# tsy935/eeg-gnn-ssl

Measured on AMD Instinct MI355X. Metric: EEG clips/sec (60s, 19ch, K=2, 2-layer x64) fwd+bwd, higher is better.
Workload: dtype f32

## Files before the change

### eeg_gnn_ssl_amd/csrc/api.cpp

```cpp
#include <algorithm>
#include <atomic>
#include <cmath>
#include <cstdarg>
#include <cstdio>
#include <cstring>

#include <string>
#include <vector>

#include "../../include/eeg_dcrnn.h"
#include "../../include/eeg_dcrnn_dev.h"
#include "../../include/eeg_dcrnn_prof.h"
#include "kernels_decoder.h"
#include "diffuse_launch.h"
#include "kernels_diffuse.h"
#include "kernels_eval.h"
#include "kernels_moments.h"
#include "kernels_scan.h"
#include "kernels_resample.h"
#include "kernels_edf.h"
#include "kernels_occlude.h"
#include "kernels_data.h"
#include "kernels_records.h"
#include "kernels_feat.h"
// ... 674 lines not shown
                                 void* stream) {
    if (eeg_dcrnn_spectral_pack_floats(Fin, H, M, N) == 0)
        return fail("pack_cell_spectral: input_dim=%d rnn_units=%d hop matrices=%d nodes=%d: the spectral form exists for 64 units", Fin, H, M, N);
    if (Wg == nullptr || Wc == nullptr || basis == nullptr || spack == nullptr) return fail("pack_cell_spectral: null pointer");
    if (launch_spec_pack(Wg, Wc, basis, Fin, H, M, N, spack, S_(stream))) return fail("pack_cell_spectral: launch failed");
    return check_launch("pack_cell_spectral");
}
int eeg_dcrnn_pack_cells(int n_cells, const float* const* Wg, const float* const* bg, const float* const* Wc, const float* const* bc,
                         const int32_t* Fin, int H, int M, float* const* packs, const float* basis, int N, float* const* spacks,
                         void* stream) {
    if (n_cells < 1 || n_cells > 4) return fail("pack_cells: %d cells (1..4 per launch)", n_cells);
    if (Wg == nullptr || bg == nullptr || Wc == nullptr || bc == nullptr || Fin == nullptr || packs == nullptr) return fail("pack_cells: null pointer table");
    if (!seq_h_supported(H)) return fail("pack_cells: rnn_units=%d unsupported", H);
    if (!seq_m_supported(M)) return fail("pack_cells: num hop matrices M=%d unsupported (1,2,3,4,5,7)", M);
    if ((basis == nullptr) != (spacks == nullptr)) return fail("pack_cells: the per-frequency packs need the basis block and their output table");
    int fin[4];
    for (int c = 0; c < n_cells; ++c) {
        fin[c] = Fin[c];
        if (fin[c] < 4 || fin[c] % 4 != 0) return fail("pack_cells: input dim %d of cell %d must be a positive multiple of 4", fin[c], c);
        if (Wg[c] == nullptr || bg[c] == nullptr || Wc[c] == nullptr || bc[c] == nullptr || packs[c] == nullptr || (spacks != nullptr && spacks[c] == nullptr))
            return fail("pack_cells: null pointer in the tables of cell %d", c);
        if (spacks != nullptr && eeg_dcrnn_spectral_pack_floats(fin[c], H, M, N) == 0)
            return fail("pack_cells: input_dim=%d rnn_units=%d hop matrices=%d nodes=%d: the spectral form exists for 64 units", fin[c], H, M, N);
    }
    if (launch_pack_cells(n_cells, Wg, bg, Wc, bc, fin, H, M, packs, basis, N, spacks, S_(stream))) return fail("pack_cells: launch failed");
    return check_launch("pack_cells");
}
int eeg_dcrnn_spectral_ok(const eeg_layer_dims* d, int need_dx) {
    if (!layer_dims_positive(d) || d->p_batched) return 0;
    if (d->x_planes_ready && d->Fin != d->H) return 0;
    if (check_dims(d->N, d->H, d->Fin, d->M)) return 0;
    return spec_supported(d->T, d->B, d->N, d->H, d->Fin, d->M, need_dx) ? 1 : 0;
}

int eeg_dcrnn_batch_major_ok(const eeg_layer_dims* d) {
    if (!diffuse_streams(diffuse_call(false, d->p_batched, d->T * d->B, d->B, d->N, d->Fin, d->M))) return 0;
    const int R = d->T * d->B * d->N;
    const GemmKnobs k = gemm_knobs();
    return (nn_dma_applies(d->Fin, R, 3 * d->H, k) && tn_dma_applies(d->Fin, 3 * d->H, k)) ? 2 : 1;
}

int eeg_dcrnn_layer_fwd(const eeg_layer_dims* d, const float* X, float* Xtm, const float* h0, const float* P,
                        const float* pack, float* planes, float* Hext, float* Rs, float* Us, float* Cs, float* RHs,
                        float* Hplanes, float* RHplanes, float* ws, void* stream) {
    if (check_dims(d->N, d->H, d->Fin, d->M)) return 1;
    if (d->T < 1 || d->B < 1) return fail("layer_fwd: empty sequence/batch (T=%d, B=%d)", d->T, d->B);
    const bool save = Rs != nullptr;
    if (save != (Us != nullptr) || save != (Cs != nullptr) || save != (RHs != nullptr))
        return fail("layer_fwd: Rs/Us/Cs/RHs must be all NULL or all non-NULL");
    hipStream_t st = S_(stream);
    const int S = d->T * d->B, R = S * d->N, H = d->H, M = d->M, Fin = d->Fin;
    const size_t state = (size_t)d->B * d->N * H;
    CellPack p = make_cell_pack(Fin, H, M);
    if (h0 != nullptr && h0 != Hext && copy_floats(Hext, h0, state, st)) return 1;
    const size_t xs = d->x_plane_stride > 0 ? (size_t)d->x_plane_stride : (size_t)R * Fin;
    BtMap bt;
    if (d->x_batch_major) {
        if (Xtm != nullptr || d->x_planes_ready) return fail("layer_fwd: x_batch_major excludes Xtm and x_planes_ready");
        if (d->spectral == nullptr && eeg_dcrnn_batch_major_ok(d) != 2) return fail("layer_fwd: x_batch_major is not available for this shape (eeg_dcrnn_batch_major_ok)");
        bt.T = d->T; bt.B = d->B; bt.N = d->N;
    }
    float* XW = ws;
    if (d->spectral != nullptr) {
        if (!eeg_dcrnn_spectral_ok(d, 0)) return fail("layer_fwd: the spectral form does not cover this shape (eeg_dcrnn_spectral_ok)");
        if (Xtm != nullptr || d->spack == nullptr) return fail("layer_fwd: spectral excludes Xtm and needs spack");
        if ((Hplanes != nullptr) != (RHplanes != nullptr)) return fail("layer_fwd: Hplanes/RHplanes must be both NULL or both non-NULL");
        const SpecPack sp = make_spec_pack(Fin, H, M, d->N);
        const int N = d->N, Sp = spec_rows(S), SpE = d->B + Sp;
        const size_t xgs = d->x_plane_stride > 0 ? (size_t)d->x_plane_stride : (size_t)Sp * Fin;
        float* Yh = ws + (size_t)R * 3 * H;
        if (!d->x_planes_ready && spec_mix(1, X, d->spectral, N, d->T, d->B, Fin, d->x_batch_major ? 1 : 0, planes, st, "spec_mix_x")) return 1;
        const SpecNnPlan nn = spec_nn_plan(Fin, Sp, N, sp.nct_x, num_cus(), spec_knobs());
        if (spec_plan_error("layer_fwd (spectral x-part)", nn.error)) return 1;
        const bool regs = nn.kind == SpecNnKind::Regs;
        if (launch_spec_nn(nn, planes, xgs, Fin, Sp, N, d->spack + (regs ? sp.sxr : sp.sxq), regs ? sp.sxr_stride : sp.sxq_stride, Yh, st, "gemm_nn_xw",
                           pack + p.bias, d->spectral + spec_csum_offset(N))) return fail("gemm_nn (spectral): launch failed");
        SeqFwdArgs a{XW, h0 != nullptr ? Hext : nullptr, P, d->p_batched, pack + p.bhg, pack + p.bhc, Hext + state, Rs, Us, Cs, RHs, nullptr, nullptr,
                     (size_t)0, d->T, d->B, N, d->act, seq_probe_arg(st)};
        SeqCall call = seq_fwd_call(H, M, N, d->T, d->B, 0, a.probe);
        call.spectral = true; call.Sp = Sp; call.SpE = SpE;
        const SeqPlan plan = seq_fwd_plan(call);
        if (plan.kind == SeqKind::TwoWaveSpec) {
            a.XW = Yh; a.Hpl = Hplanes; a.RHpl = RHplanes; a.spec_U = d->spectral; a.spec_Sp = Sp; a.spec_SpE = SpE;
            if (seq_fwd(H, M, plan, a, st)) return 1;
            if (Hplanes != nullptr) {
                if (launch_spec_zero_rows(Hplanes, N, (d->T + 1) * d->B, SpE, H, st)) return fail("spec_zero_rows: launch failed");
                if (launch_spec_zero_pad(RHplanes, N, S, H, st)) return fail("spec_zero_pad: launch failed");
            }
        } else {
            if (spec_mix(0, Yh, d->spectral, N, d->T, d->B, 3 * H, 0, XW, st, "spec_mix_y")) return 1;
            if (seq_fwd(H, M, plan, a, st)) return 1;
            if (Hplanes != nullptr) {
                if (spec_mix(1, Hext, d->spectral, N, d->T + 1, d->B, H, 0, Hplanes, st, "spec_mix_h", SpE)) return 1;
                if (spec_mix(1, RHs, d->spectral, N, d->T, d->B, H, 0, RHplanes, st, "spec_mix_h")) return 1;
            }
        }
        return check_launch("layer_fwd (spectral)");
    } else if (d->x_planes_ready) {
        if (Xtm != nullptr) return fail("layer_fwd: x_planes_ready excludes a batch-major input");
    } else {
        if (diffuse_fwd(X, P, d->p_batched, S, d->B, d->N, Fin, M, planes, st, xs, d->x_batch_major ? 2 : (Xtm != nullptr ? 1 : 0), Xtm)) return 1;
        if (Xtm != nullptr) X = Xtm;
    }
    SegPtrs segs;
    for (int m = 0; m < kMaxM; ++m) segs.p[m] = m == 0 ? X : (m < M ? planes + (size_t)(m - 1) * xs : nullptr);
    const bool bf3 = d->pack3 != nullptr && pack3_supported(Fin, H, M);
    const Pack3 q = make_pack3(Fin, H, M);
    const NnCall cxw = nn_call(M, Fin, R, 3 * H / 16, 3 * H, 3 * H, bt, p.has_bxq, bf3 ? q.xw_nct : 0);
    if (gemm_nn(gemm_nn_plan(cxw), cxw, segs, NnRhs{pack + p.bx, pack + p.bxq, bf3 ? d->pack3 + q.xw : nullptr}, pack + p.bias, XW, st, "gemm_nn_xw", bt)) return 1;
    if ((Hplanes != nullptr) != (RHplanes != nullptr)) return fail("layer_fwd: Hplanes/RHplanes must be both NULL or both non-NULL");
    SeqFwdArgs a{XW, h0 != nullptr ? Hext : nullptr, P, d->p_batched, pack + p.bhg, pack + p.bhc, Hext + state, Rs, Us, Cs, RHs, Hplanes, RHplanes,
                 (size_t)(d->T + 1) * state, d->T, d->B, d->N, d->act, seq_probe_arg(st)};
    return seq_fwd(H, M, seq_fwd_plan(seq_fwd_call(H, M, d->N, d->T, d->B, a.plane_stride, a.probe)), a, st);
}

size_t eeg_dcrnn_layer_bwd_ws_floats(const eeg_layer_dims* d, int need_dx) { return layer_dims_positive(d) ? bwd_ws(d, need_dx).total : 0; }

int eeg_dcrnn_layer_bwd(const eeg_layer_dims* d, const float* X, const float* P, const float* pack,
                        const float* planes, const float* Hext, const float* Rs, const float* Us, const float* Cs,
                        const float* RHs, const float* Hplanes, const float* RHplanes, const float* dHseq,
                        const float* d_at_end, const float* d_at_len,
                        const int64_t* lengths, float* dX, float* dh0, float* dWg, float* dbg, float* dWc,
                        float* dbc, float* ws, void* stream) {
    if (check_dims(d->N, d->H, d->Fin, d->M)) return 1;
    if (d->T < 1 || d->B < 1) return fail("layer_bwd: empty sequence/batch (T=%d, B=%d)", d->T, d->B);
    hipStream_t st = S_(stream);
    const int S = d->T * d->B, R = S * d->N, H = d->H, M = d->M, Fin = d->Fin, N = d->N;
    const size_t state = (size_t)d->B * N * H;
    CellPack p = make_cell_pack(Fin, H, M);
    BwdWs w = bwd_ws(d, dX != nullptr);
    float* dXW = ws + w.dxw;
    float* dbias = ws + w.dbias;
    SeqBwdArgs a{Hext + state, Hext, Rs, Us, Cs, dHseq, d_at_end, d_at_len,
                 reinterpret_cast<const long long*>(lengths), P, d->p_batched, pack + p.b1, pack + p.b2,
                 dXW, dh0, dbias, d->T, d->B, N, d->act, seq_probe_arg(st)};
    SeqCall call = seq_bwd_call(H, M, N, d->T, d->B, a.probe);
    call.spectral = d->spectral != nullptr; call.Sp = spec_rows(S); call.SpE = d->B + spec_rows(S);
    const SeqPlan plan = seq_bwd_plan(call);
    const bool dyh_done = plan.kind == SeqKind::TwoWaveSpec;
    if (dyh_done) { a.spec_U = d->spectral; a.dYh = ws + w.dyh; a.spec_Sp = call.Sp; }
    if (seq_bwd(H, M, plan, a, st)) return 1;
    const size_t xs = d->x_plane_stride > 0 ? (size_t)d->x_plane_stride : (size_t)R * Fin;
    BtMap bt;
    if (d->x_batch_major) {
        if (d->spectral == nullptr && eeg_dcrnn_batch_major_ok(d) != 2) return fail("layer_bwd: x_batch_major is not available for this shape");
        bt.T = d->T; bt.B = d->B; bt.N = N;
    }
    if (d->spectral != nullptr) {
        if (!eeg_dcrnn_spectral_ok(d, dX != nullptr)) return fail("layer_bwd: the spectral form does not cover this shape (eeg_dcrnn_spectral_ok)");
        if (d->spack == nullptr) return fail("layer_bwd: spectral needs spack");
        if ((Hplanes != nullptr) != (RHplanes != nullptr)) return fail("layer_bwd: Hplanes/RHplanes must be both NULL or both non-NULL");
        const SpecPack sp = make_spec_pack(Fin, H, M, N);
        const int Sp = spec_rows(S), SpE = d->B + Sp;
        float* dYh = ws + w.dyh;
        if (dyh_done) {
            if (launch_spec_zero_pad(dYh, N, S, 3 * H, st)) return fail("spec_zero_pad: launch failed");
        } else if (spec_mix(1, dXW, d->spectral, N, d->T, d->B, 3 * H, 0, dYh, st, "spec_mix_dy")) return 1;
        const float *hh = Hplanes, *rhh = RHplanes;
        size_t hh_gs = (size_t)SpE * H;
        if (hh == nullptr) {
            if (spec_mix(1, Hext, d->spectral, N, d->T, d->B, H, 0, ws + w.hplanes, st, "spec_mix_h")) return 1;
            if (spec_mix(1, RHs, d->spectral, N, d->T, d->B, H, 0, ws + w.rhplanes, st, "spec_mix_h")) return 1;
            hh = ws + w.hplanes; rhh = ws + w.rhplanes; hh_gs = 0;
        }
        if (cell_weight_grads_spectral(d, planes, xs_spec(d), hh, hh_gs, rhh, dYh, ws + w.partial, w, dWg, dWc, st, dbias, dbg, dbc)) return 1;
        if (dX != nullptr) {
// ... 1304 lines not shown
```

### eeg_gnn_ssl_amd/csrc/kernels_seq.h

```cpp
#pragma once
#include "common.h"
#include "lds_diffuse.h"

namespace eeg {

constexpr int seq_nks(int N) { return N <= 20 ? 5 : 8; }
constexpr bool seq_has_two_wave(int H, int M, int nks) { return H == 64 && nks == 5 && M <= 3; }
constexpr bool seq_has_spec(int H, int M, int nks) { return seq_has_two_wave(H, M, nks) && M >= 2; }
constexpr bool seq_has_probe(int H, int M, int nks) { return kDevBuild && H == 64 && M == 3 && nks == 5; }
constexpr bool seq_has_stream(int H, int M) { return H == 64 && M <= 5; }

template <int H, int M>
struct SeqGeom {
    static constexpr int KA = M * H, KAP = lds_stride_x(KA), KS = KA / 4;
    static constexpr int KG = M * 2 * H, KGP = lds_stride_x(KG), KSG = KG / 4;
    static constexpr int NGT = 2 * H / 16, NCT = H / 16;
    static constexpr int GT = ceil_div(NGT, 4), CT = ceil_div(NCT, 4);
};
constexpr size_t seq_fwd_lds_floats(int H, int M) { return (size_t)(M - 1) * kPFloats + 2 * 32 * lds_stride_x(M * H); }
constexpr size_t seq_fwd2_lds_floats(int H, int M, bool spec) {
    return seq_fwd_lds_floats(H, M) + 16 * 64 + (spec ? 3 * 16 * 64 + 4 * 64 + 4 * (M * H / 4 / 4) * 256 : 0);
}
constexpr size_t seq_bwd_lds_floats(int H, int M, int rows) {
    return (size_t)(M - 1) * kPFloats + (size_t)rows * (lds_stride_x(M * H) + lds_stride_x(M * 2 * H));
// ... 428 lines not shown
                    f32x4 rh = rg * ld4(A + lds_sw(node[nt], col, KAP));
                    rh = valid[nt] ? rh : zero4;
                    st4(A2 + lds_sw(node[nt], col, KAP), rh);
                    if (save && valid[nt]) {
                        wbuf_st4(bR, oh[i][nt], 0u, rg);
                        wbuf_st4(bRH, oh[i][nt], 0u, rh);
                        wbuf_st4(bU, oh[i][nt], 0u, u);
                    }
                }
            }
        }
        pp.mark(2);
        diffuse_own(A2, RHpl, t);
        pp.mark(7);
        EEG_LDS_BARRIER();
        pp.mark(3);
        if (t + 1 < T) fetch_xw(t + 1);

        mfma_nodes32<CT, KS, REM4, 0, 0, false, false, REM4>(A2, KAP, lane, lr, lg, wc, ac);
        pp.mark(4);
        const wbuf_t bH = make_wbuf(Hseq + s * N * H), bC = make_wbuf((save ? Cs : Hseq) + s * N * H);
#pragma unroll
        for (int i = 0; i < CT; ++i) {
            const int ct = wave + 4 * i;
            if (ct < NCT) {
                const int col = ct * 16 + 4 * lg;
#pragma unroll
                for (int nt = 0; nt < 2; ++nt) {
                    if (REM4 && nt == 1) {
                        const float u1 = ug[i][1][0], h1 = A[l1[i]];
                        const float c1 = act == 0 ? tanhf_(ac[i][1][0]) : fmaxf(ac[i][1][0], 0.f);
                        const float hn1 = valid1 ? u1 * h1 + (1.f - u1) * c1 : 0.f;
                        A[l1[i]] = hn1;
                        if (valid1) {
                            wbuf_st1(bH, oh[i][1], 0u, hn1);
                            if (save) wbuf_st1(bC, oh[i][1], 0u, c1);
                        }
                        continue;
                    }
                    const f32x4 u = ug[i][nt], h = ld4(A + lds_sw(node[nt], col, KAP));
                    const f32x4 c = act == 0 ? tanh4_(ac[i][nt]) : relu4_(ac[i][nt]);
                    f32x4 hn = u * h + (1.f - u) * c;
                    hn = valid[nt] ? hn : zero4;
                    st4(A + lds_sw(node[nt], col, KAP), hn);
                    if (valid[nt]) {
                        wbuf_st4(bH, oh[i][nt], 0u, hn);
                        if (save) wbuf_st4(bC, oh[i][nt], 0u, c);
                    }
                }
            }
        }
        pp.mark(5);
        if (t + 1 < T || Hpl != nullptr) diffuse_own(A, Hpl, t + 1);
        pp.mark(6);
    }
    }
    pp.dump(probe, 0);
}

template <int H, int M, int NKS, bool PROBE = false, bool SPEC = false>
__global__ __launch_bounds__(512, 1) void seq_fwd2_kernel(
    const float* __restrict__ XW, const float* __restrict__ h0, const float* __restrict__ P, int p_batched,
    const float* __restrict__ bhg, const float* __restrict__ bhc,
    float* __restrict__ Hseq, float* __restrict__ Rs, float* __restrict__ Us, float* __restrict__ Cs,
    float* __restrict__ RHs, float* __restrict__ Hpl, float* __restrict__ RHpl, size_t plane_stride,
    int T, int B, int N, int act, long long* probe, const float* __restrict__ spec_U = nullptr, int spec_Sp = 0, int spec_SpE = 0) {
    using G = SeqGeom<H, M>;
    PhaseProbe<PROBE> pp;
    pp.start();
    static_assert(G::CT == 1 && NKS == 5, "one column tile per wave, second node tile on the 4x4x1 MFMA");
    constexpr int KAP = G::KAP, KS = G::KS, NGT = G::NGT, NCT = G::NCT, UST = 64;
    EEG_DYN_SMEM(sm);
    float* Pl = sm;
    float* A = Pl + (M - 1) * kPFloats;
    float* A2 = A + 32 * KAP;
    const int tid = threadIdx.x, lane = tid & 63, wave8 = SPEC ? wave_uniform(tid >> 6) : (tid >> 6), role = wave8 >> 2, wave = wave8 & 3;
    const int lr = lane & 15, lg = lane >> 4;
    float* U = A2 + 32 * KAP;
    float* XR = U + 16 * UST;
    float* XC = XR + 16 * UST;
    float* XRr = XC + 2 * 16 * UST;
    float* W1L = XRr + 4 * 64;
    const bool save = Rs != nullptr;
    const int ct = wave;
    const wbuf_t bH = make_wbuf(Hseq), bR = make_wbuf(save ? Rs : Hseq), bU = make_wbuf(save ? Us : Hseq),
                 bC = make_wbuf(save ? Cs : Hseq), bRH = make_wbuf(save ? RHs : Hseq);

    float w0[1][KS], w1[1][KS];
#pragma unroll
    for (int ks = 0; ks < KS; ++ks) w0[0][ks] = bhg[((size_t)ks * NGT + (role == 0 ? ct : NCT + ct)) * 64 + lane];
    if (!SPEC || role == 0) {
#pragma unroll
        for (int ks = 0; ks < KS; ++ks) w1[0][ks] = bhc[((size_t)ks * NCT + ct) * 64 + lane];
    } else {
#pragma unroll
        for (int q = 0; q < KS / 4; ++q) {
            f32x4 v;
#pragma unroll
            for (int j = 0; j < 4; ++j) v[j] = bhc[((size_t)(4 * q + j) * NCT + ct) * 64 + lane];
            st4(W1L + (ct * (KS / 4) + q) * 256 + 4 * lane, v);
        }
    }
    auto clip = [&](const int b, auto ROLE_T) __attribute__((always_inline)) {
    constexpr int ROLE_C = decltype(ROLE_T)::value;
    __syncthreads();
    for (int e = tid; e < 2 * 32 * KAP; e += 512) A[e] = 0.f;
    lds_load_polys(Pl, P, p_batched ? b : 0, M, N);
    __syncthreads();
    if (h0 != nullptr) {
        for (int e = tid; e < N * H; e += 512) A[lds_sw(e / H, e % H, KAP)] = h0[(size_t)b * N * H + e];
    } else {
        for (int e = tid; e < N * H; e += 512) (Hseq - (size_t)B * N * H)[(size_t)b * N * H + e] = 0.f;
    }
    __syncthreads();

    const bool valid[2] = {lr < N, 16 + lr < N};
    const int nodec[2] = {valid[0] ? lr : N - 1, valid[1] ? 16 + lr : N - 1};
    const f32x4 zero4 = {0.f, 0.f, 0.f, 0.f};
    const int col = ct * 16 + 4 * lg;
    const int oxw0 = nodec[0] * (3 * H) + col, oh0 = nodec[0] * H + col;
    const int node1 = 16 + lg, col1 = ct * 16 + lr;
    const bool valid1 = node1 < N;
    const int oxw1 = (valid1 ? node1 : N - 1) * (3 * H) + col1, oh1 = (valid1 ? node1 : N - 1) * H + col1;
    const int l1 = lds_sw(node1, col1, KAP);
    if (ROLE_C < 0 ? role == 0 : ROLE_C == 0) {
        EEG_SETPRIO(3);
        float pf[poly_slots<M, NKS>()][NKS];
        load_poly_frags<M, NKS, false>(Pl, pf, lr, lg);
        auto diffuse_own = [&](float* buf, float* planes, int t) {
            EEG_WAVE_SYNC();
            float* g = (!SPEC && planes != nullptr) ? planes + ((size_t)t * B + b) * N * H : nullptr;
            lds_diffuse_tile<M, NKS>(buf, KAP, ct * 16, H, pf, lr, lg, g, plane_stride, N, true);
        };
        diffuse_own(A, Hpl, 0);
        f32x4 nxr0 = zero4, nxc = zero4;
        float nxr1 = 0.f;
        auto fetch_xw = [&](int t) {
            if constexpr (SPEC) return;
            const wbuf_t bx = make_wbuf(XW + ((size_t)t * B + b) * N * (3 * H));
            nxr0 = wbuf_ld4(bx, oxw0, 0u);
            nxr1 = wbuf_ld(bx, oxw1, 0u);
            nxc = wbuf_ld4(bx, oxw0 + 2 * H, 0u);
        };
        fetch_xw(0);
        pp.stamp(1);
        pp.last = PROBE ? cycle_now() : 0;
        ClockSample cs;
        const bool cs_me = !PROBE && b == 0 && tid == 0;
        cs.begin(probe, cs_me);
        constexpr int QSA = KS / 4 / M;
        f32x4 rc[5] = {zero4, zero4, zero4, zero4, zero4};
        f32x4 ra = zero4;
        bool pre_r = false;
        for (int t = 0; t < T; ++t) {
            const size_t s = (size_t)t * B + b;
            f32x4 ar[1][2] = {{nxr0, (f32x4){nxr1, 0.f, 0.f, 0.f}}}, ac[1][2] = {{nxc, zero4}};
            const unsigned so = (unsigned)(s * N * H);
            EEG_LDS_BARRIER();
            pp.mark(0);
            if constexpr (SPEC) {
                ar[0][0] = ld4(XR + lds_sw(lr, col, UST));
                ar[0][1][0] = XRr[ct * 64 + lane];
                if (M > 1 && pre_r) ra += ar[0][0];
            }

            if (M > 1 && pre_r) {
                ar[0][0] = ra;
                mfma_nodes32<1, KS, true, 0, 0, false, true, true, (M > 1 ? QSA : 0)>(A, KAP, lane, lr, lg, w0, ar, rc);
            } else
                mfma_nodes32<1, KS, true, 0, 0, false, true, true>(A, KAP, lane, lr, lg, w0, ar);
            pp.mark(1);
            {
                const f32x4 rg = sigmoid4_(ar[0][0]);
                f32x4 rh = rg * ld4(A + lds_sw(lr, col, KAP));
                rh = valid[0] ? rh : zero4;
                st4(A2 + lds_sw(lr, col, KAP), rh);
                const float rg1 = sigmoidf_(ar[0][1][0]);
                const float rh1 = valid1 ? rg1 * A[l1] : 0.f;
                A2[l1] = rh1;
                if (save && valid[0]) {
                    wbuf_st4(bR, oh0, so, rg);
                    wbuf_st4(bRH, oh0, so, rh);
                }
                if (save && valid1) {
                    wbuf_st1(bR, oh1, so, rg1);
                    wbuf_st1(bRH, oh1, so, rh1);
                }
            }
            pp.mark(2);
            diffuse_own(A2, RHpl, t);
            pp.mark(7);
            EEG_LDS_BARRIER();
            pp.mark(3);
            if (t + 1 < T) fetch_xw(t + 1);
            if constexpr (SPEC) ac[0][0] = ld4(XC + (t & 1) * (16 * UST) + lds_sw(lr, col, UST));
            mfma_nodes32<1, KS, true, 1>(A2, KAP, lane, lr, lg, w1, ac);
            pp.mark(4);
            {
                const f32x4 u = ld4(U + lds_sw(lr, col, UST)), h = ld4(A + lds_sw(lr, col, KAP));
                const f32x4 c = act == 0 ? tanh4_(ac[0][0]) : relu4_(ac[0][0]);
                f32x4 hn = u * h + (1.f - u) * c;
                hn = valid[0] ? hn : zero4;
                st4(A + lds_sw(lr, col, KAP), hn);
                if (valid[0]) {
                    wbuf_st4(bH, oh0, so, hn);
                    if (save) wbuf_st4(bC, oh0, so, c);
                }
            }
            pp.mark(5);
            EEG_LDS_BARRIER();
            if (t + 1 < T || (!SPEC && Hpl != nullptr)) diffuse_own(A, Hpl, t + 1);
            pre_r = M > 1 && t + 1 < T;
            if (pre_r) {
                ra = SPEC ? zero4 : nxr0;
                rc[0] = rc[1] = rc[2] = rc[3] = rc[4] = zero4;
                f32x4 rr4[4] = {zero4, zero4, zero4, zero4};
                mfma_tile_quads<KS, 0, QSA>(A, KAP, lane, lr, lg, w0[0], ra, rc[4], rr4);
                rc[0] = rr4[0]; rc[1] = rr4[1]; rc[2] = rr4[2]; rc[3] = rr4[3];
            }
            pp.mark(6);
        }
        cs.end(probe, cs_me);
        pp.stamp(2);
    } else {
        f32x4 nxu0 = zero4;
        float nxu1 = 0.f, nxc1 = 0.f;
        float ux[NKS], ux4[NKS], ut[NKS], ut4[NKS], yv[3][NKS];
        const unsigned vyb = (unsigned)lg * (unsigned)spec_Sp * (3 * H) + ct * 16 + lr;
        const unsigned vy4 = (unsigned)(16 + lg < N ? 16 + lg : N - 1) * (unsigned)spec_Sp * (3 * H) + ct * 16 + lr;
        const wbuf_t bY = make_wbuf(XW), bHh = make_wbuf(Hpl != nullptr ? Hpl : Hseq), bRHh = make_wbuf(RHpl != nullptr ? RHpl : Hseq);
        const unsigned oe0 = (unsigned)lr * (unsigned)spec_SpE * H + col, oe1 = (unsigned)node1 * (unsigned)spec_SpE * H + col1;
        const unsigned or0 = (unsigned)lr * (unsigned)spec_Sp * H + col, or1 = (unsigned)node1 * (unsigned)spec_Sp * H + col1;
        if constexpr (SPEC) {
            load_spec_frags<NKS>(spec_U, N, lane, ut, ut4);
#pragma unroll
            for (int ks = 0; ks < NKS; ++ks) {
                const int i = 4 * ks + lg, j4 = 16 + (lane & 3);
                ux[ks] = (i < N && lr < N) ? spec_U[lr * N + i] : 0.f;
                ux4[ks] = (i < N && j4 < N) ? spec_U[j4 * N + i] : 0.f;
            }
        }
        auto fetch_y = [&](int t) {
            const unsigned so = (unsigned)(((size_t)t * B + b) * (3 * H));
#pragma unroll
            for (int g = 0; g < 3; ++g)
#pragma unroll
                for (int ks = 0; ks < NKS; ++ks)
                    yv[g][ks] = ks < 4 ? wbuf_ld(bY, vyb + g * H, so + (unsigned)(4 * ks) * (unsigned)spec_Sp * (3 * H)) : wbuf_ld(bY, vy4 + g * H, so);
        };
        auto xw_mix = [&](int tn) {
            f32x4 acc[3] = {zero4, zero4, zero4}, rem[3] = {zero4, zero4, zero4}, rem2[3] = {zero4, zero4, zero4};
#pragma unroll
            for (int ks = 0; ks < NKS; ++ks)
#pragma unroll
                for (int g = 0; g < 3; ++g) acc[g] = mfma16(yv[g][ks], ux[ks], acc[g]);
#pragma unroll
            for (int ks = 0; ks < NKS; ++ks)
#pragma unroll
                for (int g = 0; g < 3; ++g) {
                    if (ks & 1) rem2[g] = mfma4(ux4[ks], yv[g][ks], rem2[g]);
                    else rem[g] = mfma4(ux4[ks], yv[g][ks], rem[g]);
                }
            f32x4 t0 = rem[0] + rem2[0], t1 = rem[1] + rem2[1], t2 = rem[2] + rem2[2];
            EEG_PIN(t0); EEG_PIN(t1); EEG_PIN(t2);
            st4(XR + lds_sw(lr, col, UST), acc[0]);
            st4(XC + (tn & 1) * (16 * UST) + lds_sw(lr, col, UST), acc[2]);
            XRr[ct * 64 + lane] = rem4_reduce(t0);
            nxu0 = acc[1];
            nxu1 = rem4_reduce(t1);
            nxc1 = rem4_reduce(t2);
        };
        auto export_tile = [&](const float* tile, wbuf_t out, unsigned o0, unsigned o1, unsigned row) {
            const float* const tl[1] = {tile};
            const int strd[1] = {KAP}, scol[1] = {ct * 16}, gcol[1] = {0};
            spec_mix_tiles_out<NKS, 1>(tl, strd, scol, gcol, ut, ut4, lr, lg, out, o0, o1, row * H, valid[0], valid1);
        };
        auto fetch_x = [&](int t) {
            if constexpr (SPEC) { fetch_y(t); return; }
            const wbuf_t bx = make_wbuf(XW + ((size_t)t * B + b) * N * (3 * H));
            nxu0 = wbuf_ld4(bx, oxw0 + H, 0u);
            nxu1 = wbuf_ld(bx, oxw1 + H, 0u);
            nxc1 = wbuf_ld(bx, oxw1 + 2 * H, 0u);
        };
        fetch_x(0);
        if constexpr (SPEC) {
            xw_mix(0);
        }
        constexpr int QS = KS / 4 / M;
        f32x4 ua = zero4, ub = zero4, urem[4] = {zero4, zero4, zero4, zero4};
        float ux1 = 0.f;
        bool pre = false;
        for (int t = 0; t < T; ++t) {
            const size_t s = (size_t)t * B + b;
            f32x4 au[1][2] = {{nxu0, (f32x4){nxu1, 0.f, 0.f, 0.f}}}, ac[1][2] = {{zero4, (f32x4){nxc1, 0.f, 0.f, 0.f}}};
            const unsigned so = (unsigned)(s * N * H);
            EEG_LDS_BARRIER();
            if (!pre) {
                ua = nxu0; ub = zero4; ux1 = nxu1;
                urem[0] = urem[1] = urem[2] = urem[3] = zero4;
            }
            if (t + 1 < T) fetch_x(t + 1);
            if (!pre) mfma_tile_quads<KS, 0, QS>(A, KAP, lane, lr, lg, w0[0], ua, ub, urem);
            mfma_tile_quads<KS, QS, KS / 4>(A, KAP, lane, lr, lg, w0[0], ua, ub, urem);
            {
                f32x4 tt = (urem[0] + urem[1]) + (urem[2] + urem[3]);
                EEG_PIN(tt);
                au[0][0] = ua + ub;
                au[0][1][0] = ux1 + rem4_reduce(tt);
            }
            float u1;
            {
                const f32x4 u0 = sigmoid4_(au[0][0]);
                u1 = sigmoidf_(au[0][1][0]);
                st4(U + lds_sw(lr, col, UST), u0);
                if (save && valid[0]) wbuf_st4(bU, oh0, so, u0);
            }
            if constexpr (SPEC) {
                if (Hpl != nullptr) export_tile(A, bHh, oe0, oe1, (unsigned)s);
            }
            EEG_LDS_BARRIER();
            if constexpr (SPEC) ac[0][1][0] += mfma_rem4_ldsw<KS>(A2, KAP, lane, lg, W1L + ct * (KS / 4) * 256);
            else mfma_nodes32<1, KS, true, 2, 0, false, false, true>(A2, KAP, lane, lr, lg, w1, ac);
            {
                const float h1 = A[l1];
                const float c1 = act == 0 ? tanhf_(ac[0][1][0]) : fmaxf(ac[0][1][0], 0.f);
                const float hn1 = valid1 ? u1 * h1 + (1.f - u1) * c1 : 0.f;
                A[l1] = hn1;
                if (valid1) {
                    wbuf_st1(bH, oh1, so, hn1);
                    if (save) {
                        wbuf_st1(bC, oh1, so, c1);
                        wbuf_st1(bU, oh1, so, u1);
                    }
                }
            }
            if constexpr (SPEC) {
                if (RHpl != nullptr) export_tile(A2, bRHh, or0, or1, (unsigned)s);
            }
            EEG_LDS_BARRIER();
#ifdef EEG_X_BPRE
            pre = t + 1 < T;
#else
            pre = !SPEC && t + 1 < T;
#endif
            if constexpr (SPEC) {
                if (!pre && t + 1 < T) xw_mix(t + 1);
            }
            if (pre) {
                ua = SPEC ? zero4 : nxu0; ub = zero4; ux1 = SPEC ? 0.f : nxu1;
                urem[0] = urem[1] = urem[2] = urem[3] = zero4;
                mfma_tile_quads<KS, 0, QS>(A, KAP, lane, lr, lg, w0[0], ua, ub, urem);
                if constexpr (SPEC) {
                    xw_mix(t + 1);
                    ua += nxu0;
                    ux1 = nxu1;
                }
            }
        }
        if constexpr (SPEC) {
            if (Hpl != nullptr) export_tile(A, bHh, oe0, oe1, (unsigned)((size_t)T * B + b));
        }
    }
    };
    if constexpr (SPEC) {
        if (role == 0) { for (int b = blockIdx.x; b < B; b += gridDim.x) clip(b, SeqIdx<0>()); }
        else { for (int b = blockIdx.x; b < B; b += gridDim.x) clip(b, SeqIdx<1>()); }
    } else {
        for (int b = blockIdx.x; b < B; b += gridDim.x) clip(b, SeqIdx<-1>());
// ... 227 lines not shown
        mfma_nodes32<CT, KSG, REM4, 0, 0, false, false, REM4>(EG, KGP, lane, lr, lg, w2, dhn);
        pp.mark(5);
#pragma unroll
        for (int i = 0; i < CT; ++i) {
            dh[i][0] = dhn[i][0];
            dh[i][1] = dhn[i][1];
        }
    }

    __syncthreads();
    float* red = EG;
    float* red1 = EG + 3 * H * 16;
#pragma unroll
    for (int i = 0; i < CT; ++i) {
        if (own[i]) {
            const int col = (wave + 4 * i) * 16 + 4 * lg;
            if (dh0 != nullptr) {
                if (valid[0]) st4(dh0 + boff + node[0] * H + col, dh[i][0]);
                if (REM4) {
                    if (valid1) dh0[boff + node1 * H + (wave + 4 * i) * 16 + lr] = dh[i][1][0];
                } else if (valid[1]) {
                    st4(dh0 + boff + node[1] * H + col, dh[i][1]);
                }
            }
#pragma unroll
            for (int r = 0; r < 4; ++r) {
                red[(0 * H + col + r) * 16 + lr] = sb_r[i][r];
                red[(1 * H + col + r) * 16 + lr] = sb_u[i][r];
                red[(2 * H + col + r) * 16 + lr] = sb_c[i][r];
            }
            if (REM4) {
                const int c1 = (wave + 4 * i) * 16 + lr;
                red1[(0 * H + c1) * 4 + lg] = sb1_r[i];
                red1[(1 * H + c1) * 4 + lg] = sb1_u[i];
                red1[(2 * H + c1) * 4 + lg] = sb1_c[i];
            }
        }
    }
    __syncthreads();
    for (int j = tid; j < 3 * H; j += 256) {
        float sacc = 0.f;
#pragma unroll
        for (int q = 0; q < 16; ++q) sacc += red[j * 16 + q];
        if (REM4) sacc += (red1[j * 4] + red1[j * 4 + 1]) + (red1[j * 4 + 2] + red1[j * 4 + 3]);
        dbias_part[(size_t)b * 3 * H + j] = sacc;
    }
    }
    pp.dump(probe, 8);
}

template <int H, int M, int NKS, bool PROBE = false, bool SPEC = false>
__global__ __launch_bounds__(512, 1) void seq_bwd2_kernel(
    const float* __restrict__ Hseq, const float* __restrict__ h0, const float* __restrict__ Rs,
    const float* __restrict__ Us, const float* __restrict__ Cs, const float* __restrict__ dHseq,
    const float* __restrict__ d_at_end, const float* __restrict__ d_at_len, const long long* __restrict__ lengths,
    const float* __restrict__ P, int p_batched, const float* __restrict__ b1p, const float* __restrict__ b2p,
    float* __restrict__ dXW, float* __restrict__ dh0, float* __restrict__ dbias_part, int T, int B, int N, int act,
    long long* probe, const float* __restrict__ spec_U = nullptr, float* __restrict__ dYh = nullptr, int spec_Sp = 0) {
    using G = SeqGeom<H, M>;
    static_assert(G::CT == 1 && NKS == 5, "one column tile per wave, second node tile on the 4x4x1 MFMA");
    constexpr int KAP = G::KAP, KS = G::KS, KGP = G::KGP, KSG = G::KSG, NCT = G::NCT, ROWS = 32, DPS = 20;
    constexpr int kCoefTile = 5 * 256 + 256 + 64;
    PhaseProbe<PROBE> pp;
    pp.start();
    EEG_DYN_SMEM(sm);
    float* Pl = sm;
    float* EC = Pl + (M - 1) * kPFloats;
    float* EG = EC + ROWS * KAP;
    const int tid = threadIdx.x, lane = tid & 63, wave8 = tid >> 6, role = wave8 >> 2, ct = wave8 & 3;
    const int lr = lane & 15, lg = lane >> 4;
    float* DP = EG + ROWS * KGP + ct * (20 * DPS);
    float* CF0 = EG + ROWS * KGP + 4 * 20 * DPS + ct * kCoefTile;
    constexpr int kZero = ROWS * (KAP + KGP) + 4 * 20 * DPS + 2 * 4 * kCoefTile;
    static_assert((size_t)(M - 1) * kPFloats + kZero == seq_bwd2_lds_floats(H, M), "the launch plan sizes the dynamic LDS by seq_bwd2_lds_floats");
    const int node[2] = {lr, 16 + lr};
    const bool valid[2] = {lr < N, 16 + lr < N};
    const int nodec[2] = {valid[0] ? lr : N - 1, valid[1] ? 16 + lr : N - 1};
    const f32x4 zero4 = {0.f, 0.f, 0.f, 0.f};
    const int col = ct * 16 + 4 * lg;
    const int node1 = 16 + lg, col1 = ct * 16 + lr;
    const bool valid1 = node1 < N;
    const int odp0 = lr * DPS + 4 * lg, odp1 = node1 * DPS + lr;
    auto cf_buf = [&](int t) { return CF0 + (t & 1) * (4 * kCoefTile); };

    if (role == 1) {
        float w2[1][KSG];
#pragma unroll
        for (int ks = 0; ks < KSG; ++ks) w2[0][ks] = b2p[((size_t)ks * NCT + ct) * 64 + lane];
        const int oh0 = nodec[0] * H + col, oh1 = (valid1 ? node1 : N - 1) * H + col1;
        const int orow[2] = {lr, valid[1] ? 16 + lr : 16};
        for (int b = blockIdx.x; b < B; b += gridDim.x) {
            __syncthreads();
            for (int e = tid; e < kZero; e += 512) EC[e] = 0.f;
            lds_load_polys(Pl, P, p_batched ? b : 0, M, N);
            int t_len = -1;
            if (d_at_len != nullptr) {
                t_len = lengths != nullptr ? (int)lengths[b] - 1 : T - 1;
                t_len = t_len < 0 ? 0 : (t_len >= T ? T - 1 : t_len);
            }
            const size_t tstride = (size_t)B * N * H, boff = (size_t)b * N * H;
            f32x4 nh, nr, nu, nc, ng;
            float nh1, nr1, nu1, nc1, ng1;
            const wbuf_t bH = make_wbuf(Hseq), bH0 = make_wbuf(h0 != nullptr ? h0 : Hseq), bR = make_wbuf(Rs), bU = make_wbuf(Us),
                         bC = make_wbuf(Cs), bG = make_wbuf(dHseq != nullptr ? dHseq : Hseq);
            auto fetch = [&](int t) {
                const unsigned so = (unsigned)((size_t)t * tstride + boff);
                nh = t > 0 ? wbuf_ld4(bH, oh0, so - (unsigned)tstride) : (h0 != nullptr ? wbuf_ld4(bH0, oh0, (unsigned)boff) : zero4);
                nr = wbuf_ld4(bR, oh0, so);
                nu = wbuf_ld4(bU, oh0, so);
                nc = wbuf_ld4(bC, oh0, so);
                nh1 = t > 0 ? wbuf_ld(bH, oh1, so - (unsigned)tstride) : (h0 != nullptr ? wbuf_ld(bH0, oh1, (unsigned)boff) : 0.f);
                nr1 = wbuf_ld(bR, oh1, so);
                nu1 = wbuf_ld(bU, oh1, so);
                nc1 = wbuf_ld(bC, oh1, so);
                f32x4 g = dHseq != nullptr ? wbuf_ld4(bG, oh0, so) : zero4;
                float g1 = dHseq != nullptr ? wbuf_ld(bG, oh1, so) : 0.f;
                if (d_at_end != nullptr && t == T - 1) { g += ld4(d_at_end + boff + oh0); g1 += d_at_end[boff + oh1]; }
                if (t == t_len) { g += ld4(d_at_len + boff + oh0); g1 += d_at_len[boff + oh1]; }
                ng = g;
                ng1 = g1;
            };
            f32x4 gx;
            float gx1;
            auto coef = [&](int t_of) {
                float* CF = cf_buf(t_of) + 4 * lane;
                {
                    const f32x4 h = nh, u = nu, c = nc, r = nr;
                    f32x4 kC, kU, hr1;
#pragma unroll
                    for (int e = 0; e < 4; ++e) {
                        const float one_u = 1.f - u[e];
                        kC[e] = act == 0 ? one_u * (1.f - c[e] * c[e]) : (c[e] > 0.f ? one_u : 0.f);
                        kU[e] = (h[e] - c[e]) * u[e] * one_u;
                        hr1[e] = h[e] * r[e] * (1.f - r[e]);
                    }
                    st4(CF + 0 * 256, kC);
                    st4(CF + 1 * 256, kU);
                    st4(CF + 2 * 256, u);
                    st4(CF + 3 * 256, hr1);
                    st4(CF + 4 * 256, r);
                    gx = ng;
                }
                {
                    const float one_u = 1.f - nu1;
                    const float kC1 = act == 0 ? one_u * (1.f - nc1 * nc1) : (nc1 > 0.f ? one_u : 0.f);
                    st4(CF + 5 * 256, (f32x4){kC1, (nh1 - nc1) * nu1 * one_u, nu1, nh1 * nr1 * (1.f - nr1)});
                    CF[6 * 256 - 3 * lane] = nr1;
                    gx1 = ng1;
                }
            };
            fetch(T - 1);
            __syncthreads();
            coef(T - 1);
            if (T > 1) fetch(T - 2);
            st4(DP + odp0, gx);
            DP[odp1] = gx1;
            f32x4 sb_r = zero4, sb_u = zero4, sb_c = zero4;
            EEG_LDS_BARRIER();
            for (int t = T - 1; t >= 0; --t) {
                if (t < T - 1) {
                    sb_r += ld4(EG + lds_sw(orow[0], col, KGP));
                    if (valid[1]) sb_r += ld4(EG + lds_sw(orow[1], col, KGP));
                }
                if (t > 0) {
                    coef(t - 1);
                    if (t > 1) fetch(t - 2);
                }
                EEG_LDS_BARRIER();
                f32x4 acc[1][2] = {{zero4, zero4}};
                mfma_nodes32<1, KSG, true, 0, 2, true, true, true>(EG, KGP, lane, lr, lg, w2, acc);
                sb_c += ld4(EC + lds_sw(orow[0], col, KAP));
                sb_u += ld4(EG + lds_sw(orow[0], H + col, KGP));
                if (valid[1]) {
                    sb_c += ld4(EC + lds_sw(orow[1], col, KAP));
                    sb_u += ld4(EG + lds_sw(orow[1], H + col, KGP));
                }
                EEG_LDS_BARRIER();
                EEG_SETPRIO(3);
                mfma_nodes32<1, KSG, true, 0, 1, true, true, true>(EG, KGP, lane, lr, lg, w2, acc);
                EEG_SETPRIO(0);
                if (t > 0) { acc[0][0] += gx; acc[0][1][0] += gx1; }
                st4(DP + odp0, acc[0][0]);
                DP[odp1] = acc[0][1][0];
                EEG_LDS_BARRIER();
            }
            sb_r += ld4(EG + lds_sw(orow[0], col, KGP));
            if (valid[1]) sb_r += ld4(EG + lds_sw(orow[1], col, KGP));
            __syncthreads();
            float* red = EG;
#pragma unroll
            for (int r = 0; r < 4; ++r) {
                red[(0 * H + col + r) * 16 + lr] = sb_r[r];
                red[(1 * H + col + r) * 16 + lr] = sb_u[r];
                red[(2 * H + col + r) * 16 + lr] = sb_c[r];
            }
            __syncthreads();
            for (int j = tid - 256; j < 3 * H; j += 256) {
                float sacc = 0.f;
#pragma unroll
                for (int q = 0; q < 16; ++q) sacc += red[j * 16 + q];
                dbias_part[(size_t)b * 3 * H + j] = sacc;
            }
        }
        return;
    }
    float w1[1][KS];
#pragma unroll
    for (int ks = 0; ks < KS; ++ks) w1[0][ks] = b1p[((size_t)ks * NCT + ct) * 64 + lane];
    for (int b = blockIdx.x; b < B; b += gridDim.x) {
    __syncthreads();
    for (int e = tid; e < kZero; e += 512) EC[e] = 0.f;
    lds_load_polys(Pl, P, p_batched ? b : 0, M, N);
    __syncthreads();
    EEG_SETPRIO(3);
    float pf[poly_slots<M, NKS>()][NKS];
    load_poly_frags<M, NKS, true>(Pl, pf, lr, lg);
    float uf[NKS], u4[NKS];
    if constexpr (SPEC) load_spec_frags<NKS>(spec_U, N, lane, uf, u4);
    const wbuf_t bY = make_wbuf(SPEC ? dYh : dXW);
    const unsigned oy0 = (unsigned)lr * (unsigned)spec_Sp * (3 * H) + col, oy1 = (unsigned)node1 * (unsigned)spec_Sp * (3 * H) + col1;
    const int oxw0 = node[0] * (3 * H) + col, oxw1 = node1 * (3 * H) + col1;
    const int lc1 = lds_sw(node1, col1, KAP), lg1 = lds_sw(node1, col1, KGP), lu1 = lds_sw(node1, H + col1, KGP);
    const size_t boff = (size_t)b * N * H;
    f32x4 dhn = zero4;
    float dhn1 = 0.f;
    EEG_LDS_BARRIER();
    const wbuf_t bX = make_wbuf(dXW);
    pp.stamp(1);
    pp.last = PROBE ? cycle_now() : 0;
    ClockSample cs;
    const bool cs_me = !PROBE && b == 0 && tid == 0;
    cs.begin(probe == nullptr ? nullptr : probe + 2, cs_me);
    for (int t = T - 1; t >= 0; --t) {
        const unsigned sx = (unsigned)(((size_t)t * B + b) * N * (3 * H));
        f32x4 hr1, rg;
        float hr1_1, rg1;
        {
            const float* CF = cf_buf(t) + 4 * lane;
            const f32x4 g = valid[0] ? dhn + ld4(DP + odp0) : zero4;
            const f32x4 dC = g * ld4(CF + 0 * 256), du_ = g * ld4(CF + 1 * 256);
            st4(EC + lds_sw(lr, col, KAP), dC);
            st4(EG + lds_sw(lr, H + col, KGP), du_);
            if (!SPEC && valid[0]) {
                wbuf_st4(bX, oxw0 + 2 * H, sx, dC);
                wbuf_st4(bX, oxw0 + H, sx, du_);
            }
            dhn = g * ld4(CF + 2 * 256);
            hr1 = ld4(CF + 3 * 256);
            rg = ld4(CF + 4 * 256);
            const float g1 = valid1 ? dhn1 + DP[odp1] : 0.f;
            const f32x4 k1 = ld4(CF + 5 * 256);
            const float dC1 = g1 * k1[0], du1 = g1 * k1[1];
            EC[lc1] = dC1;
            EG[lu1] = du1;
            if (!SPEC && valid1) {
                wbuf_st1(bX, oxw1 + 2 * H, sx, dC1);
                wbuf_st1(bX, oxw1 + H, sx, du1);
            }
            dhn1 = g1 * k1[2];
            hr1_1 = k1[3];
            rg1 = CF[6 * 256 - 3 * lane];
        }
        pp.mark(0);
        EEG_WAVE_SYNC();
        lds_diffuse_tile<M, NKS, ROWS>(EC, KAP, ct * 16, H, pf, lr, lg);
        lds_diffuse_tile<M, NKS, ROWS>(EG, KGP, H + ct * 16, 2 * H, pf, lr, lg);
        pp.mark(7);
        EEG_LDS_BARRIER();
        pp.mark(1);
        f32x4 acc[1][2] = {{zero4, zero4}};
        mfma_nodes32<1, KS, true, 0, 0, false, false, true>(EC, KAP, lane, lr, lg, w1, acc);
        pp.mark(2);
        {
            const f32x4 drh = acc[0][0];
            const f32x4 dR = drh * hr1;
            dhn += drh * rg;
            st4(EG + lds_sw(lr, col, KGP), dR);
            if (!SPEC && valid[0]) wbuf_st4(bX, oxw0, sx, dR);
            const float drh1 = acc[0][1][0], dR1 = drh1 * hr1_1;
            dhn1 += drh1 * rg1;
            EG[lg1] = dR1;
            if (!SPEC && valid1) wbuf_st1(bX, oxw1, sx, dR1);
        }
        pp.mark(3);
        EEG_WAVE_SYNC();
        lds_diffuse_tile<M, NKS, ROWS>(EG, KGP, ct * 16, 2 * H, pf, lr, lg);
        EEG_LDS_BARRIER();
        pp.mark(4);
        EEG_SETPRIO(0);
        if constexpr (SPEC) {
            const float* const tl[3] = {EG, EG, EC};
            const int strd[3] = {KGP, KGP, KAP}, scol[3] = {ct * 16, H + ct * 16, ct * 16}, gcol[3] = {0, H, 2 * H};
            const unsigned row = (unsigned)t * (unsigned)B + (unsigned)b;
            EEG_WAVE_SYNC();
            spec_mix_tiles_out<NKS, 3>(tl, strd, scol, gcol, uf, u4, lr, lg, bY, oy0, oy1, row * (3 * H), valid[0], valid1);
        }
        EEG_LDS_BARRIER();
        EEG_SETPRIO(3);
        pp.mark(6);
    }
    cs.end(probe == nullptr ? nullptr : probe + 2, cs_me);
    pp.stamp(2);
    __syncthreads();
    if (dh0 != nullptr) {
        if (valid[0]) st4(dh0 + boff + lr * H + col, dhn + ld4(DP + odp0));
        if (valid1) dh0[boff + node1 * H + col1] = dhn1 + DP[odp1];
    }
    __syncthreads();
    }
// ... 5 lines not shown
```

### eeg_gnn_ssl_amd/csrc/lds_diffuse.h

```cpp
#pragma once
#include "common.h"

namespace eeg {

__device__ __forceinline__ void lds_load_polys(float* Pl, const float* __restrict__ P, int g, int M, int N) {
    const int total = (M - 1) * kPFloats;
    for (int e = threadIdx.x; e < total; e += blockDim.x) {
        const int m1 = e / kPFloats, r = (e % kPFloats) / kPStride, c = e % kPStride;
        float v = 0.f;
        if (r < N && c < N) v = P[(((size_t)g * (M - 1) + m1) * N + r) * N + c];
        Pl[e] = v;
    }
}

template <bool ADJ, int UNR = 4>
__device__ __forceinline__ void lds_diffuse_tiles(float* buf, int stride, int src_off, int dst_off,
                                                  int dst_step, int W, const float* Pl, int M, int N,
                                                  int rows_limit) {
    const int lane = threadIdx.x & 63, wave = threadIdx.x >> 6, nwaves = blockDim.x >> 6;
    const int nct = W / 16, nks = ceil_div(N, 4);
    const int ntiles = (M - 1) * 2 * nct;
    const int lr = lane & 15, lg = lane >> 4;
    for (int t0 = wave; t0 < ntiles; t0 += nwaves * UNR) {
        f32x4 acc[UNR];
        int aoff[UNR], boff[UNR], doff[UNR], row0[UNR];
        bool ok[UNR];
#pragma unroll
        for (int u = 0; u < UNR; ++u) {
            const int t = t0 + u * nwaves;
            ok[u] = t < ntiles;
            const int tt = ok[u] ? t : t0;
            const int ct = tt % nct, rt = (tt / nct) & 1, m1 = tt / (2 * nct);
            aoff[u] = m1 * kPFloats + (ADJ ? (lg * kPStride + rt * 16 + lr) : ((rt * 16 + lr) * kPStride + lg));
            boff[u] = lg * stride + src_off + ct * 16 + lr;
            row0[u] = rt * 16 + 4 * lg;
            doff[u] = row0[u] * stride + dst_off + m1 * dst_step + ct * 16 + lr;
            acc[u] = (f32x4){0.f, 0.f, 0.f, 0.f};
        }
        for (int ks = 0; ks < nks; ++ks) {
#pragma unroll
            for (int u = 0; u < UNR; ++u) {
                const float a = Pl[aoff[u] + (ADJ ? 4 * ks * kPStride : 4 * ks)];
                const float b = buf[boff[u] + 4 * ks * stride];
                acc[u] = mfma16(a, b, acc[u]);
            }
        }
#pragma unroll
        for (int u = 0; u < UNR; ++u) {
            if (ok[u]) {
#pragma unroll
                for (int r = 0; r < 4; ++r)
                    if (row0[u] + r < rows_limit) buf[doff[u] + r * stride] = acc[u][r];
            }
        }
    }
}

template <int M, int NKS>
constexpr int poly_chains() { return NKS == 5 ? (M - 1) + (M - 1 + 3) / 4 : (M - 1) * 2; }
template <int M, int NKS>
constexpr int poly_slots() { return poly_chains<M, NKS>() > 0 ? poly_chains<M, NKS>() : 1; }

template <int M, int NKS, bool ADJ>
__device__ __forceinline__ void load_poly_frags(const float* Pl, float (&pf)[poly_slots<M, NKS>()][NKS], int lr, int lg) {
    if constexpr (NKS == 5) {
#pragma unroll
        for (int c = 0; c < M - 1; ++c)
#pragma unroll
            for (int ks = 0; ks < NKS; ++ks)
                pf[c][ks] = ADJ ? Pl[c * kPFloats + (4 * ks + lg) * kPStride + lr] : Pl[c * kPFloats + lr * kPStride + 4 * ks + lg];
#pragma unroll
        for (int pc = 0; pc < (M - 1 + 3) / 4; ++pc) {
            const int hop = 4 * pc + (lr >> 2), r = 16 + (lr & 3);
#pragma unroll
            for (int ks = 0; ks < NKS; ++ks) {
                float v = 0.f;
                if (hop < M - 1) v = ADJ ? Pl[hop * kPFloats + (4 * ks + lg) * kPStride + r] : Pl[hop * kPFloats + r * kPStride + 4 * ks + lg];
                pf[M - 1 + pc][ks] = v;
            }
        }
    } else {
#pragma unroll
        for (int c = 0; c < (M - 1) * 2; ++c) {
            const int m1 = c >> 1, rt = c & 1;
#pragma unroll
            for (int ks = 0; ks < NKS; ++ks)
                pf[c][ks] = ADJ ? Pl[m1 * kPFloats + (4 * ks + lg) * kPStride + rt * 16 + lr]
                                : Pl[m1 * kPFloats + (rt * 16 + lr) * kPStride + 4 * ks + lg];
        }
    }
}

template <int M, int NKS, int ROWS = 32>
__device__ __forceinline__ void lds_diffuse_tile(float* buf, int stride, int src_col, int slot_w,
                                                 const float (&pf)[poly_slots<M, NKS>()][NKS], int lr, int lg,
                                                 float* __restrict__ gout = nullptr, size_t gplane = 0, int n_nodes = 0,
// ... 73 lines not shown
```

Before: 128,800.

## Overlap per-clip polynomial and h0 loads with first-step fetches in seq kernels

Per-clip staging of the diffusion polynomials and initial hidden state now runs in two steps. Global loads are issued into registers first (PolyShare and an hv array), alongside the first XW/x fetches, and are written to LDS only after the tiles are cleared with 16-byte stores. The change also skips the initial diffusion when h0 is null, moves the W1 LDS staging to the first clip with buffer loads, and drops the RH sequence store when RH planes already hold it. The aim is to hide global-load latency behind barrier-separated setup. The cost is more registers, which may lower occupancy or cause spills.

```diff
diff --git a/eeg_gnn_ssl_amd/csrc/api.cpp b/eeg_gnn_ssl_amd/csrc/api.cpp
--- a/eeg_gnn_ssl_amd/csrc/api.cpp
+++ b/eeg_gnn_ssl_amd/csrc/api.cpp
@@ -780,6 +780,7 @@
         const SeqPlan plan = seq_fwd_plan(call);
         if (plan.kind == SeqKind::TwoWaveSpec) {
             a.XW = Yh; a.Hpl = Hplanes; a.RHpl = RHplanes; a.spec_U = d->spectral; a.spec_Sp = Sp; a.spec_SpE = SpE;
+            if (RHplanes != nullptr) a.RHs = nullptr;
             if (seq_fwd(H, M, plan, a, st)) return 1;
             if (Hplanes != nullptr) {
                 if (launch_spec_zero_rows(Hplanes, N, (d->T + 1) * d->B, SpE, H, st)) return fail("spec_zero_rows: launch failed");
diff --git a/eeg_gnn_ssl_amd/csrc/kernels_seq.h b/eeg_gnn_ssl_amd/csrc/kernels_seq.h
--- a/eeg_gnn_ssl_amd/csrc/kernels_seq.h
+++ b/eeg_gnn_ssl_amd/csrc/kernels_seq.h
@@ -534,9 +534,10 @@
     float* XRr = XC + 2 * 16 * UST;
     float* W1L = XRr + 4 * 64;
     const bool save = Rs != nullptr;
+    const bool save_rh = save && RHs != nullptr;
     const int ct = wave;
     const wbuf_t bH = make_wbuf(Hseq), bR = make_wbuf(save ? Rs : Hseq), bU = make_wbuf(save ? Us : Hseq),
-                 bC = make_wbuf(save ? Cs : Hseq), bRH = make_wbuf(save ? RHs : Hseq);
+                 bC = make_wbuf(save ? Cs : Hseq), bRH = make_wbuf(save_rh ? RHs : Hseq);
 
     float w0[1][KS], w1[1][KS];
 #pragma unroll
@@ -544,27 +545,40 @@
     if (!SPEC || role == 0) {
 #pragma unroll
         for (int ks = 0; ks < KS; ++ks) w1[0][ks] = bhc[((size_t)ks * NCT + ct) * 64 + lane];
-    } else {
-#pragma unroll
-        for (int q = 0; q < KS / 4; ++q) {
-            f32x4 v;
-#pragma unroll
-            for (int j = 0; j < 4; ++j) v[j] = bhc[((size_t)(4 * q + j) * NCT + ct) * 64 + lane];
-            st4(W1L + (ct * (KS / 4) + q) * 256 + 4 * lane, v);
-        }
     }
     auto clip = [&](const int b, auto ROLE_T) __attribute__((always_inline)) {
     constexpr int ROLE_C = decltype(ROLE_T)::value;
-    __syncthreads();
-    for (int e = tid; e < 2 * 32 * KAP; e += 512) A[e] = 0.f;
-    lds_load_polys(Pl, P, p_batched ? b : 0, M, N);
-    __syncthreads();
-    if (h0 != nullptr) {
-        for (int e = tid; e < N * H; e += 512) A[lds_sw(e / H, e % H, KAP)] = h0[(size_t)b * N * H + e];
-    } else {
-        for (int e = tid; e < N * H; e += 512) (Hseq - (size_t)B * N * H)[(size_t)b * N * H + e] = 0.f;
-    }
-    __syncthreads();
+    constexpr int NHV = ceil_div(20 * H, 512);
+    PolyShare<M, 512> pv;
+    float hv[NHV];
+    auto request_tiles = [&]() {
+        pv.request(P, p_batched ? b : 0, N);
+        if (h0 != nullptr) {
+            const wbuf_t b0 = make_wbuf(h0 + (size_t)b * N * H);
+#pragma unroll
+            for (int i = 0; i < NHV; ++i) {
+                const int e = tid + 512 * i;
+                hv[i] = e < N * H ? wbuf_ld(b0, (unsigned)e, 0u) : 0.f;
+            }
+        }
+    };
+    auto stage_tiles = [&]() {
+        EEG_LDS_BARRIER();
+        for (int e = 4 * tid; e < 2 * 32 * KAP; e += 4 * 512) st4(A + e, (f32x4){0.f, 0.f, 0.f, 0.f});
+        EEG_LDS_BARRIER();
+        pv.store(Pl);
+        if (h0 != nullptr) {
+#pragma unroll
+            for (int i = 0; i < NHV; ++i) {
+                const int e = tid + 512 * i;
+                if (e < N * H) A[lds_sw(e / H, e % H, KAP)] = hv[i];
+            }
+        } else {
+            for (int e = tid; e < N * H; e += 512) (Hseq - (size_t)B * N * H)[(size_t)b * N * H + e] = 0.f;
+        }
+        EEG_LDS_BARRIER();
+    };
+    static_assert(((M - 1) * kPFloats) % 4 == 0 && (2 * 32 * KAP) % 4 == 0, "the tiles are cleared with 16-byte stores");
 
     const bool valid[2] = {lr < N, 16 + lr < N};
     const int nodec[2] = {valid[0] ? lr : N - 1, valid[1] ? 16 + lr : N - 1};
@@ -576,15 +590,6 @@
     const int oxw1 = (valid1 ? node1 : N - 1) * (3 * H) + col1, oh1 = (valid1 ? node1 : N - 1) * H + col1;
     const int l1 = lds_sw(node1, col1, KAP);
     if (ROLE_C < 0 ? role == 0 : ROLE_C == 0) {
-        EEG_SETPRIO(3);
-        float pf[poly_slots<M, NKS>()][NKS];
-        load_poly_frags<M, NKS, false>(Pl, pf, lr, lg);
-        auto diffuse_own = [&](float* buf, float* planes, int t) {
-            EEG_WAVE_SYNC();
-            float* g = (!SPEC && planes != nullptr) ? planes + ((size_t)t * B + b) * N * H : nullptr;
-            lds_diffuse_tile<M, NKS>(buf, KAP, ct * 16, H, pf, lr, lg, g, plane_stride, N, true);
-        };
-        diffuse_own(A, Hpl, 0);
         f32x4 nxr0 = zero4, nxc = zero4;
         float nxr1 = 0.f;
         auto fetch_xw = [&](int t) {
@@ -594,7 +599,18 @@
             nxr1 = wbuf_ld(bx, oxw1, 0u);
             nxc = wbuf_ld4(bx, oxw0 + 2 * H, 0u);
         };
+        request_tiles();
         fetch_xw(0);
+        stage_tiles();
+        EEG_SETPRIO(3);
+        float pf[poly_slots<M, NKS>()][NKS];
+        load_poly_frags<M, NKS, false>(Pl, pf, lr, lg);
+        auto diffuse_own = [&](float* buf, float* planes, int t) {
+            EEG_WAVE_SYNC();
+            float* g = (!SPEC && planes != nullptr) ? planes + ((size_t)t * B + b) * N * H : nullptr;
+            lds_diffuse_tile<M, NKS>(buf, KAP, ct * 16, H, pf, lr, lg, g, plane_stride, N, true);
+        };
+        if (h0 != nullptr || (!SPEC && Hpl != nullptr)) diffuse_own(A, Hpl, 0);
         pp.stamp(1);
         pp.last = PROBE ? cycle_now() : 0;
         ClockSample cs;
@@ -632,11 +648,11 @@
                 A2[l1] = rh1;
                 if (save && valid[0]) {
                     wbuf_st4(bR, oh0, so, rg);
-                    wbuf_st4(bRH, oh0, so, rh);
+                    if (save_rh) wbuf_st4(bRH, oh0, so, rh);
                 }
                 if (save && valid1) {
                     wbuf_st1(bR, oh1, so, rg1);
-                    wbuf_st1(bRH, oh1, so, rh1);
+                    if (save_rh) wbuf_st1(bRH, oh1, so, rh1);
                 }
             }
             pp.mark(2);
@@ -683,6 +699,16 @@
         const wbuf_t bY = make_wbuf(XW), bHh = make_wbuf(Hpl != nullptr ? Hpl : Hseq), bRHh = make_wbuf(RHpl != nullptr ? RHpl : Hseq);
         const unsigned oe0 = (unsigned)lr * (unsigned)spec_SpE * H + col, oe1 = (unsigned)node1 * (unsigned)spec_SpE * H + col1;
         const unsigned or0 = (unsigned)lr * (unsigned)spec_Sp * H + col, or1 = (unsigned)node1 * (unsigned)spec_Sp * H + col1;
+        const bool first_clip = SPEC && b == (int)blockIdx.x;
+        f32x4 wl[KS / 4];
+        if (first_clip) {
+            const wbuf_t bW = make_wbuf(bhc);
+#pragma unroll
+            for (int q = 0; q < KS / 4; ++q)
+#pragma unroll
+                for (int j = 0; j < 4; ++j) wl[q][j] = wbuf_ld(bW, (unsigned)(ct * 64 + lane), (unsigned)((4 * q + j) * NCT * 64));
+        }
+        request_tiles();
         if constexpr (SPEC) {
             load_spec_frags<NKS>(spec_U, N, lane, ut, ut4);
 #pragma unroll
@@ -735,7 +761,12 @@
             nxc1 = wbuf_ld(bx, oxw1 + 2 * H, 0u);
         };
         fetch_x(0);
+        stage_tiles();
         if constexpr (SPEC) {
+            if (first_clip) {
+#pragma unroll
+                for (int q = 0; q < KS / 4; ++q) st4(W1L + (ct * (KS / 4) + q) * 256 + 4 * lane, wl[q]);
+            }
             xw_mix(0);
         }
         constexpr int QS = KS / 4 / M;
@@ -1129,6 +1160,10 @@
     const bool valid1 = node1 < N;
     const int odp0 = lr * DPS + 4 * lg, odp1 = node1 * DPS + lr;
     auto cf_buf = [&](int t) { return CF0 + (t & 1) * (4 * kCoefTile); };
+    static_assert(((M - 1) * kPFloats) % 4 == 0 && kZero % 4 == 0, "the tiles are cleared with 16-byte stores");
+    auto clear_tiles = [&]() {
+        for (int e = 4 * tid; e < kZero; e += 4 * 512) st4(EC + e, zero4);
+    };
 
     if (role == 1) {
         float w2[1][KSG];
@@ -1137,14 +1172,13 @@
         const int oh0 = nodec[0] * H + col, oh1 = (valid1 ? node1 : N - 1) * H + col1;
         const int orow[2] = {lr, valid[1] ? 16 + lr : 16};
         for (int b = blockIdx.x; b < B; b += gridDim.x) {
-            __syncthreads();
-            for (int e = tid; e < kZero; e += 512) EC[e] = 0.f;
-            lds_load_polys(Pl, P, p_batched ? b : 0, M, N);
             int t_len = -1;
             if (d_at_len != nullptr) {
                 t_len = lengths != nullptr ? (int)lengths[b] - 1 : T - 1;
                 t_len = t_len < 0 ? 0 : (t_len >= T ? T - 1 : t_len);
             }
+            PolyShare<M, 512> pv;
+            pv.request(P, p_batched ? b : 0, N);
             const size_t tstride = (size_t)B * N * H, boff = (size_t)b * N * H;
             f32x4 nh, nr, nu, nc, ng;
             float nh1, nr1, nu1, nc1, ng1;
@@ -1197,7 +1231,10 @@
                 }
             };
             fetch(T - 1);
-            __syncthreads();
+            EEG_LDS_BARRIER();
+            clear_tiles();
+            EEG_LDS_BARRIER();
+            pv.store(Pl);
             coef(T - 1);
             if (T > 1) fetch(T - 2);
             st4(DP + odp0, gx);
@@ -1255,15 +1292,15 @@
 #pragma unroll
     for (int ks = 0; ks < KS; ++ks) w1[0][ks] = b1p[((size_t)ks * NCT + ct) * 64 + lane];
     for (int b = blockIdx.x; b < B; b += gridDim.x) {
-    __syncthreads();
-    for (int e = tid; e < kZero; e += 512) EC[e] = 0.f;
-    lds_load_polys(Pl, P, p_batched ? b : 0, M, N);
-    __syncthreads();
-    EEG_SETPRIO(3);
-    float pf[poly_slots<M, NKS>()][NKS];
-    load_poly_frags<M, NKS, true>(Pl, pf, lr, lg);
+    PolyShare<M, 512> pv;
+    pv.request(P, p_batched ? b : 0, N);
     float uf[NKS], u4[NKS];
     if constexpr (SPEC) load_spec_frags<NKS>(spec_U, N, lane, uf, u4);
+    EEG_LDS_BARRIER();
+    clear_tiles();
+    EEG_LDS_BARRIER();
+    pv.store(Pl);
+    EEG_SETPRIO(3);
     const wbuf_t bY = make_wbuf(SPEC ? dYh : dXW);
     const unsigned oy0 = (unsigned)lr * (unsigned)spec_Sp * (3 * H) + col, oy1 = (unsigned)node1 * (unsigned)spec_Sp * (3 * H) + col1;
     const int oxw0 = node[0] * (3 * H) + col, oxw1 = node1 * (3 * H) + col1;
@@ -1272,6 +1309,8 @@
     f32x4 dhn = zero4;
     float dhn1 = 0.f;
     EEG_LDS_BARRIER();
+    float pf[poly_slots<M, NKS>()][NKS];
+    load_poly_frags<M, NKS, true>(Pl, pf, lr, lg);
     const wbuf_t bX = make_wbuf(dXW);
     pp.stamp(1);
     pp.last = PROBE ? cycle_now() : 0;
diff --git a/eeg_gnn_ssl_amd/csrc/lds_diffuse.h b/eeg_gnn_ssl_amd/csrc/lds_diffuse.h
--- a/eeg_gnn_ssl_amd/csrc/lds_diffuse.h
+++ b/eeg_gnn_ssl_amd/csrc/lds_diffuse.h
@@ -12,6 +12,26 @@
         Pl[e] = v;
     }
 }
+template <int M, int NT>
+struct PolyShare {
+    static constexpr int kTotal = (M - 1) * kPFloats, kPer = ceil_div(kTotal, NT);
+    float v[kPer > 0 ? kPer : 1];
+    __device__ __forceinline__ void request(const float* __restrict__ P, int g, int N) {
+        const wbuf_t Pg = make_wbuf(P + (size_t)g * (M - 1) * N * N);
+#pragma unroll
+        for (int i = 0; i < kPer; ++i) {
+            const int e = (int)threadIdx.x + NT * i, m1 = e / kPFloats, r = (e % kPFloats) / kPStride, c = e % kPStride;
+            v[i] = (e < kTotal && r < N && c < N) ? wbuf_ld(Pg, (unsigned)((m1 * N + r) * N + c), 0u) : 0.f;
+        }
+    }
+    __device__ __forceinline__ void store(float* Pl) const {
+#pragma unroll
+        for (int i = 0; i < kPer; ++i) {
+            const int e = (int)threadIdx.x + NT * i;
+            if (e < kTotal) Pl[e] = v[i];
+        }
+    }
+};
 
 template <bool ADJ, int UNR = 4>
 __device__ __forceinline__ void lds_diffuse_tiles(float* buf, int stride, int src_off, int dst_off,
```

Result: no change. 130,000, median of 5 (+1.0%).
